# ZwwWayne/mmMOT

Hardware: AMD Instinct MI355X
Metric: frame-pairs/sec (fusion+affinity fwd) at N_det=64; affinity L∞ vs CPU ref (higher is better)
Workload: dtype f16x3

## Files before the change

include/mmmot_hip.h:

```cpp
#ifndef MMMOT_HIP_H
#define MMMOT_HIP_H

#include <stddef.h>
#include <stdint.h>

#ifdef __cplusplus
extern "C" {
#endif

#define MMMOT_OK 0
#define MMMOT_EINVAL (-1)

#define MMMOT_ACT_NONE 0
#define MMMOT_ACT_RELU 1
#define MMMOT_ACT_SIGMOID 2

#define MMMOT_A_PLAIN 0
#define MMMOT_A_NORM_RELU 1
#define MMMOT_A_PAIR 2

#define MMMOT_PAIR_MULTIPLY 0
#define MMMOT_PAIR_MINUS_ABS 1
#define MMMOT_PAIR_MINUS 2

// ... 101 lines not shown

int mmmot_gn_finalize(const float* part, const int* grp_tile0, const int* grp_ntiles,
                      const int* grp_count, const int* tile_nrows, int G, int ldp, int C, int NG,
                      const float* gamma, const float* beta, float eps,
                      float* sc, float* sh, void* stream);

int mmmot_segment_mean(const float* X, int ldx, int C,
                       const int* seg_start, const int* seg_count, const int* seg_stride,
                       const int* seg_group, const int* seg_div, int nseg,
                       const float* sc, const float* sh, int ldsc, int relu,
                       float* out, int ldo,
                       int hl16 ,
                       void* stream);

int mmmot_rowdot(const float* X, int ldx, int K, const float* w, float b,
                 const float* sc, const float* sh, int ldsc,
                 const int* tile_row0, const int* tile_nrows, const int* tile_group, int T,
                 int act, int use_thr, float thr,
                 float* out, const int* omap, void* stream);

int mmmot_row_layernorm(const float* X, int ldx, int C, const float* gamma, const float* beta,
                        float eps, int relu, float* Y, int ldy, int R, void* stream);

int mmmot_skippool_head(const float* P, int ldp, int C, int C4, const float* g0, const float* b0, const float* w1,
                        const float* c1, const float* g2, const float* b2, const float* w4, const float* c4,
                        const float* g5, const float* b5, float eps, float* out, int ldo, int R, void* stream);
int mmmot_pointnet_layer1(const float* X, int K, const float* W, const float* bias,
                          float* Y, float* part,
                          const int* tile_row0, const int* tile_nrows, int T, void* stream);

int mmmot_pn_mlp64(const float* X, int ldx, const float* sc, const float* sh, int ldsc, const void* W16,
                   float oscale, const float* bias, float* Y, int ldy, float* part, const int* tile_row0,
                   const int* tile_nrows, const int* tile_group, int T, int N, void* stream);

int mmmot_affine_act(const float* X, int ldx, int C, const float* sc, const float* sh, int ldsc,
                     const int* tile_row0, const int* tile_nrows, const int* tile_group, int T,
                     int act, float* Y, int ldy, void* stream);

int mmmot_fusion_combine(int mode, const float* cat, const float* Y0, int ld0,
                         const float* Y1, int ld1,
                         const float* sc0, const float* sh0, const float* sc1, const float* sh1, int ldsc,
                         const int* tile_row0, const int* tile_nrows, const int* tile_group, int T,
                         float* F, int Lt, int C, void* stream);

int mmmot_softmax_pairs(const float* logits, float* out,
                        const int* grp_row0, const int* grp_N, const int* grp_M, int G,
                        int max_nm ,
                        int mode, void* stream);

int mmmot_points_count(const float* pts, int P, int F, const double* planes, int NB, int pad_empty,
                       int* cnt, int* split, void* stream);
int mmmot_points_scatter(const float* pts, int P, int F, const double* planes, int NB, const int* cnt,
                         const int* split, float* out, int Fo, void* stream);
int mmmot_points_count_batched(const float* pts, int F, int NS, int NPOLY, int NBLK, int cnt_total,
                               const double* planes, const int* blk_sweep, const int* blk_first,
                               const int* sweep_row0, const int* poly0, const int* filt, const int* cnt_off,
                               int pad_empty, int* cnt, int* split, void* stream);
int mmmot_points_scatter_batched(const float* pts, int F, int NS, int NPOLY, int NBLK, int cnt_total,
                                 const double* planes, const int* blk_sweep, const int* blk_first,
                                 const int* sweep_row0, const int* poly0, const int* filt, const int* cnt_off,
                                 const int* cnt, const int* split, float* out, int Fo, void* stream);

int mmmot_u8_normalize(const unsigned char* u8, int N, int S, const float* mean_std, float* out, void* stream);
int mmmot_crop_resize_norm(const unsigned char* img, int H, int W, const int* boxes, int N, int S, int kmax,
                           const float* mean_std, int* work, float* out, unsigned char* out_u8, void* stream);

// ... 86 lines not shown
```

mmmot_amd/_lib.py:

```python
import ctypes
import os
import subprocess
import threading

_HERE = os.path.dirname(os.path.abspath(__file__))
CSRC = os.path.join(_HERE, 'csrc')
LIB_PATH = os.environ.get('MMMOT_LIB_PATH', os.path.join(_HERE, 'libmmmot_hip.so'))
SOURCES = ['conv3x3.hip', 'hl16_format.hip', 'conv3x3_hl16_patch.hip', 'gemm_rows.hip', 'gemm_wide.hip',
           'gemm_ares.hip', 'gemm_wres.hip', 'gemm_wreg.hip', 'pn_mlp64.hip', 'gram.hip', 'points_gather.hip', 'crop_resize.hip', 'small_kernels.hip', 'backward.hip', 'train.hip', 'train_vgg.hip', 'gemm_tn_f16.hip',
           'assign.hip', 'track_ids.hip']
HIPCC = os.environ.get('HIPCC', '/opt/rocm/bin/hipcc')
HIPFLAGS = ['--offload-arch=gfx950', '-O3', '-std=c++17', '-fPIC']

_lock = threading.Lock()
_lib = None

c_f = ctypes.c_void_p
c_i = ctypes.c_int


class GemmArgs(ctypes.Structure):
    _fields_ = [
        ('X', c_f), ('ldx', c_i),
        ('W', c_f),
        ('bias', c_f),
        ('dbias', c_f), ('rowidx', c_f), ('lddb', c_i),
        ('Y', c_f), ('ldy', c_i),
        ('part', c_f),
        ('sc', c_f), ('sh', c_f), ('ldsc', c_i),
        ('FA', c_f), ('FB', c_f), ('ldf', c_i),
        ('tile_row0', c_f), ('tile_nrows', c_f), ('tile_group', c_f),
        ('grp_row0', c_f), ('grp_M', c_f), ('grp_aoff', c_f), ('grp_boff', c_f),
        ('T', c_i), ('N', c_i), ('K', c_i),
        ('amode', c_i), ('pairop', c_i), ('act', c_i),
        ('w_hl16', c_i), ('oscale', ctypes.c_float),
        ('osc', c_f), ('osh', c_f), ('ldosc', c_i),
        ('colsum', c_f),
        ('pair_uniform32', c_i),
    ]


class GemmAresArgs(ctypes.Structure):
# ... 36 lines not shown
    'mmmot_gram_rows': [c_f, c_i, c_i, c_f, c_f, c_i, c_f, c_f, c_f, c_i, c_f, c_f, c_f],
    'mmmot_set_gram128_variant': [c_i],
    'mmmot_gn_finalize_gram': [c_f, c_f, c_f, c_f, c_f, c_i, c_i, c_f, c_f, c_i, c_f, c_f, ctypes.c_float, c_f, c_f, c_f, c_f],
    'mmmot_gn_finalize_gram_dbias': [c_f, c_f, c_f, c_f, c_f, c_i, c_f, c_f, c_i, c_f, c_f, c_i, c_i, c_f, c_f, ctypes.c_float,
                                     c_f, c_f, c_f, c_f],
    'mmmot_gn_finalize': [c_f, c_f, c_f, c_f, c_f, c_i, c_i, c_i, c_i, c_f, c_f, ctypes.c_float, c_f, c_f, c_f],
    'mmmot_segment_mean': [c_f, c_i, c_i, c_f, c_f, c_f, c_f, c_f, c_i, c_f, c_f, c_i, c_i, c_f, c_i, c_i, c_f],
    'mmmot_conv3x3_bn_relu_hl16_patch': [c_f, c_f, c_f, c_f, c_i, c_i, c_i, c_i, c_i, c_i, c_f, c_f],
    'mmmot_conv1_fused_hl16': [c_f, c_f, c_f, ctypes.c_float, c_f, c_f, c_f, c_f, c_i, c_i, c_i, c_f],
    'mmmot_conv3x3_bn_relu_hq8': [c_f, c_f, c_f, c_f, c_i, c_i, c_i, c_i, c_i, c_i, c_f, c_f],
    'mmmot_conv1_fused_u8': [c_f, ctypes.c_float, ctypes.c_float, ctypes.c_float, ctypes.c_float, ctypes.c_float,
                             ctypes.c_float, c_f, c_f, ctypes.c_float, c_f, c_f, c_f, c_f, c_i, c_i, c_i, c_i, c_f],
    'mmmot_u8_normalize': [c_f, c_i, c_i, c_f, c_f, c_f],
    'mmmot_conv1_fused_hq8': [c_f, c_f, c_f, ctypes.c_float, c_f, c_f, c_f, c_f, c_i, c_i, c_i, c_f],
    'mmmot_conv3x3_first_hl16': [c_f, c_f, c_f, c_f, c_i, c_i, c_i, c_i, c_f],
    'mmmot_set_patch_grid_limit': [c_i],
    'mmmot_set_patch_min_block': [c_i],
    'mmmot_trunk_range_read': [ctypes.POINTER(ctypes.c_uint), c_i],
    'mmmot_trunk_range_bind': [c_f],
    'mmmot_hl16_pack': [c_f, c_f, ctypes.c_long, c_f],
    'mmmot_hl16_unpack': [c_f, c_f, ctypes.c_long, c_f],
    'mmmot_hl16_pack_pow2': [c_f, c_f, ctypes.c_long, c_f, c_i, c_f],
    'mmmot_pow2_oscale': [c_f, c_i, c_f, c_i, c_f, c_i, c_f],
    'mmmot_conv3x3_raw_hl16': [c_f, c_f, c_f, c_f, c_i, c_i, c_i, c_i, c_i, c_f, c_f],
    'mmmot_hq8_pack': [c_f, c_f, ctypes.c_long, c_f],
    'mmmot_hq8_unpack': [c_f, c_f, ctypes.c_long, c_f],
    'mmmot_rowdot': [c_f, c_i, c_i, c_f, ctypes.c_float, c_f, c_f, c_i, c_f, c_f, c_f, c_i, c_i, c_i,
                     ctypes.c_float, c_f, c_f, c_f],
    'mmmot_row_layernorm': [c_f, c_i, c_i, c_f, c_f, ctypes.c_float, c_i, c_f, c_i, c_i, c_f],
    'mmmot_skippool_head': [c_f, c_i, c_i, c_i, c_f, c_f, c_f, c_f, c_f, c_f, c_f, c_f, c_f, c_f, ctypes.c_float, c_f, c_i, c_i,
                            c_f],
    'mmmot_pointnet_layer1': [c_f, c_i, c_f, c_f, c_f, c_f, c_f, c_f, c_i, c_f],
    'mmmot_pn_mlp64': [c_f, c_i, c_f, c_f, c_i, c_f, ctypes.c_float, c_f, c_f, c_i, c_f, c_f, c_f, c_f, c_i, c_i, c_f],
    'mmmot_affine_act': [c_f, c_i, c_i, c_f, c_f, c_i, c_f, c_f, c_f, c_i, c_i, c_f, c_i, c_f],
    'mmmot_fusion_combine': [c_i, c_f, c_f, c_i, c_f, c_i, c_f, c_f, c_f, c_f, c_i, c_f, c_f, c_f, c_i, c_f,
                             c_i, c_i, c_f],
    'mmmot_softmax_pairs': [c_f, c_f, c_f, c_f, c_f, c_i, c_i, c_i, c_f],
    'mmmot_points_count': [c_f, c_i, c_i, c_f, c_i, c_i, c_f, c_f, c_f],
    'mmmot_points_scatter': [c_f, c_i, c_i, c_f, c_i, c_f, c_f, c_f, c_i, c_f],
    'mmmot_crop_resize_norm': [c_f, c_i, c_i, c_f, c_i, c_i, c_i, c_f, c_f, c_f, c_f, c_f],
    'mmmot_points_count_batched': [c_f, c_i, c_i, c_i, c_i, c_i, c_f, c_f, c_f, c_f, c_f, c_f, c_f, c_i, c_f, c_f, c_f],
    'mmmot_points_scatter_batched': [c_f, c_i, c_i, c_i, c_i, c_i, c_f, c_f, c_f, c_f, c_f, c_f, c_f, c_f, c_f, c_f, c_i, c_f],
    'mmmot_selftest_mfma': [c_f, c_f, c_f, c_i, c_f],
    'mmmot_gn_bwd_partial': [c_f, c_i, c_f, c_i, c_i, c_f, c_f, c_i, c_f, c_f, c_i, c_f, c_f, c_f, c_i, c_f, c_f],
    'mmmot_gn_bwd_finalize': [c_f, c_f, c_i, c_i, c_i, c_f, c_f, c_f],
    'mmmot_gn_bwd_apply': [c_f, c_i, c_f, c_i, c_i, c_f, c_f, c_i, c_f, c_f, c_i, c_f, c_f, c_f, c_f, c_i, c_f, c_i, c_f],
    'mmmot_gemm_tn': [ctypes.POINTER(GemmTnArgs), c_f],
    'mmmot_gemm_tn_f16': [ctypes.POINTER(GemmTnArgs), c_f, c_f],
    'mmmot_absmax': [c_f, c_i, ctypes.c_long, c_i, c_f, c_f],
    'mmmot_pair_bwd': [c_f, c_i, c_f, c_i, c_f, c_i, c_i, c_f, c_f, c_f, c_f, c_f, c_f, c_f, c_i, c_i, c_i, c_f],
    'mmmot_pair_expand_bwd': [c_f, c_i, c_f, c_i, c_i, c_f, c_f, c_f, c_i, c_f, c_f, c_f, c_f, c_f],
    'mmmot_rowdot_bwd': [c_f, c_i, c_i, c_f, ctypes.c_float, c_f, c_f, c_i, c_f, c_f, c_f, c_i, c_i, c_f, c_f, c_f, c_i,
                         c_f, c_i, c_f],
    'mmmot_softmax_pairs_bwd': [c_f, c_f, c_f, c_f, c_f, c_f, c_i, c_i, c_i, c_f],
    'mmmot_fusion_c_bwd': [c_f, c_f, c_i, c_f, c_i, c_f, c_f, c_f, c_f, c_i, c_f, c_f, c_f, c_i, c_f, c_f, c_i, c_f, c_f, c_i, c_f],
    'mmmot_add_rows': [c_f, c_i, c_f, c_i, c_f, c_i, ctypes.c_long, c_i, c_f],
    'mmmot_conv3x3_raw': [c_f, c_f, c_f, c_f, c_i, c_i, c_i, c_i, c_i, c_i, c_f],
    'mmmot_rows_stats': [c_f, c_i, c_i, c_f, c_f, c_i, c_f, c_f],
    'mmmot_bn_relu_pool': [c_f, c_i, c_f, c_f, c_i, c_i, c_i, c_i, c_f, c_f],
    'mmmot_maxpool_bwd': [c_f, c_i, c_f, c_f, c_f, c_i, c_i, c_i, c_f, c_f],
    'mmmot_conv3x3_wgrad': [c_f, c_f, c_i, c_i, c_i, c_i, c_i, c_i, c_f, c_f],
    'mmmot_conv3x3_wgrad_f16': [c_f, c_f, c_i, c_i, c_i, c_i, c_i, c_i, c_f, c_f, c_f],
    'mmmot_conv3x3_first_wgrad': [c_f, c_f, c_i, c_i, c_i, c_f, c_i, c_f],
    'mmmot_rows_gather_scale': [c_f, c_i, c_f, c_f, c_f, c_i, ctypes.c_long, c_i, c_f],
    'mmmot_pointnet_layer1_bwd': [c_f, c_f, c_i, c_f, c_f, c_i, c_f, c_f],
    'mmmot_score_loss': [c_f, c_i, c_f, c_f, c_f, c_i, c_i, ctypes.c_float, c_i, ctypes.c_float, c_i, c_i, c_f, c_i, c_f,
# ... 74 lines not shown
```

mmmot_amd/engine.py:

```python
import contextlib
import itertools
import os
import threading

import numpy as np
import torch

from .ops import (ACT_NONE, ACT_RELU, ACT_SIGMOID, A_NORM_RELU, A_PAIR, A_PLAIN, FUSION_MODES, PAIR_OPS,
                  SOFTMAX_MODES)
from .range_guard import RangeGuard

POOL_INPUT = {'f32': 0, 'hl16': 1, 'hq8': 2}
EPS = 1e-5
_SERIALS = itertools.count(1)


def check_crop_side(S):
    if S < 32 or S % 2 != 0:
        raise ValueError('crop side %d is not supported: the HIP VGG trunk needs an even side >= 32; resize the crops '
                         '(mmmot_amd.crops.crop_resize_normalize)' % S)


def check_crop_layout(dets):
    if dets.dtype == torch.uint8:
        if dets.dim() != 4 or dets.shape[3] != 3 or dets.shape[1] != dets.shape[2]:
            raise ValueError('uint8 crops must be [L,S,S,3] (HWC, the output of mmmot_amd.crops.crop_resize_u8), got %s'
                             % (tuple(dets.shape),))
        S = int(dets.shape[1])
    else:
        S = int(dets.shape[-1])
    check_crop_side(S)
    return S


class Engine:
    def __init__(self, packed, ops, fusion='A', affinity_op='multiply', softmax_mode='none',
                 neg_threshold=0.0, score_arch='branch_cls', end_mode='avg', trunk=None):
        trunk = trunk or os.environ.get('MMMOT_TRUNK', 'f16x3')
        if trunk not in ('f16x3', 'f16q8', 'f32'):
            raise ValueError("trunk must be 'f16x3' (fp16 matrix cores, 3-term split), 'f16q8' (fp16 main term + "
                             "fp8 correction terms, include/mmmot_hip.h hq8) or 'f32' (exact fp32 MFMA)")
        self.trunk = trunk
        self.serial = next(_SERIALS)
        self.trunk_requested = trunk
        self.guard = RangeGuard(self)
        self.range_events = []
        self.last_out_of_range_forward = None
        self.out_of_range_window = None
        self._busy = threading.Lock()
        self._last_stream = None
        self._image_token = None
        self._pre_image = None
        ql = os.environ.get('MMMOT_Q8_LAYERS', '4,5,6,7,8,9,10,11,12')
        self.q8_layers = None if ql == 'all' else set(int(v) for v in ql.split(',') if v)
        self.pn_fused = os.environ.get('MMMOT_PN_FUSED', '1') != '0'
        self.pn_gram = os.environ.get('MMMOT_PN_GRAM', '1') != '0'
        self.pn_mlp64 = os.environ.get('MMMOT_PN_MLP64', '1') != '0'
        self.two_streams = os.environ.get('MMMOT_TWO_STREAMS', '0') == '1'
        self.pn_beside_trunk = os.environ.get('MMMOT_PN_BESIDE_TRUNK', '1') != '0'
        self._side = {}
        self.sp_fused = os.environ.get('MMMOT_SP_FUSED', '1') != '0'
        self.fuse_conv1 = os.environ.get('MMMOT_FUSE_CONV1', '1') != '0'
        self.q8_min_crop = int(os.environ.get('MMMOT_Q8_MIN_CROP', '64'))
        self.mlp = 'f32' if trunk == 'f32' else 'f16x3'
        if affinity_op not in PAIR_OPS:
            raise ValueError('unknown affinity_op %r' % (affinity_op,))
        if softmax_mode not in SOFTMAX_MODES and softmax_mode != 'none':
            softmax_mode = 'none'
        self.end_mode = end_mode
        self.P = packed
        self.ops = ops
        self.fusion = fusion
        self.affinity_op = affinity_op
        self.softmax_mode = softmax_mode
        self.neg_threshold = float(neg_threshold)
        self.score_arch = score_arch
        self.ws = {}
        self.dev = None
        self.keep = None
        self.conv_events = None

    def buf(self, name, *shape, device=None, dtype=torch.float32):
        n = 1
        for s in shape:
            n *= int(s)
        t = self.ws.get(name)
        if t is None or t.numel() < n or t.dtype != dtype or (device is not None and t.device != torch.device(device)):
            t = torch.empty(max(n, 4), dtype=dtype, device=device if device is not None else self.dev)
            self.ws[name] = t
        return t[:n].view(*shape)
# ... 137 lines not shown

    def _skippool(self, plan, s, x, hw, C, cat, fmt='f32'):
        hl16 = POOL_INPUT[fmt]
        ops, Lt, hd, T = self.ops, plan.Lt, self.P['skippool'][s], plan.det_tiles
        pooled = self.buf('sp_pool', Lt, C)
        first, second, npart = plan.crop_segments(hw)
        if second is None:
            ops.segment_mean(x, C, first, pooled, use_group=False, hl16=hl16)
        else:
            partial = self.buf('sp_partial', npart, C)
            ops.segment_mean(x, C, first, partial, use_group=False, hl16=hl16)
            ops.segment_mean(partial, C, second, pooled, use_group=False)
        if self.sp_fused and hasattr(ops, 'skippool_head'):
            ops.skippool_head(pooled, C, hd, EPS, cat[:, 128 * s:128 * (s + 1)], Lt)
            return
        ln0 = self.buf('sp_ln0', Lt, C)
        ops.row_layernorm(pooled, C, hd['g0'], hd['b0'], EPS, False, ln0, Lt)
        C4 = hd['w1'].shape[0]
        h1 = self.buf('sp_h1', Lt, C4)
        self._gemm(hd, 'w1', T, C4, C, X=ln0, bias=hd['c1'], Y=h1)
        ln1 = self.buf('sp_ln1', Lt, C4)
        ops.row_layernorm(h1, C4, hd['g2'], hd['b2'], EPS, True, ln1, Lt)
        h2 = self.buf('sp_h2', Lt, 128)
        self._gemm(hd, 'w4', T, 128, C4, X=ln1, bias=hd['c4'], Y=h2)
        ops.row_layernorm(h2, 128, hd['g5'], hd['b5'], EPS, True, cat[:, 128 * s:128 * (s + 1)], Lt)

    def pointnet(self, plan, points, cat):
        ops, pn, T, D, Pn, Lt = self.ops, self.P['pointnet'], plan.pt_tiles, plan.det_tiles, plan.P, plan.Lt
        y1 = self.buf('pn_y1', Pn, 64)
        part = self._part(T, 64)
        ops.pointnet_layer1(points, pn['w1'], pn['b1'], y1, part, T)
        sc1, sh1 = self._finalize('pn1', part, T, 64, 64, pn['g1'], pn['be1'])
        x, sc, sh = y1, sc1, sh1
        for i, (N, K) in zip((2, 3, 4), ((64, 64), (64, 64), (128, 64))):
            y = self.buf('pn_y%d' % i, Pn, N)
            part = self._part(T, N)
            if self.pn_mlp64 and self.mlp == 'f16x3' and ('w%d_h16' % i) in pn:
                ops.pn_mlp64(pn['w%d_h16' % i], pn['w%d_os' % i], T, N, x, sc, sh, pn['b%d' % i], y, part)
            else:
                self._gemm(pn, 'w%d' % i, T, N, K, X=x, bias=pn['b%d' % i], Y=y, part=part, sc=sc, sh=sh,
                           amode=A_NORM_RELU)
            sc, sh = self._finalize('pn%d' % i, part, T, N, N, pn['g%d' % i], pn['be%d' % i])
            x = y
        seg1024 = self._norm_relu_pool(plan, 'w5', '5', 128, 1024, x, sc, sh)
        self._stash('pn_seg1024', seg1024)
        dbias = self.buf('pn_dbias', Lt, 512)
        self._gemm(pn, 'wc1b', D, 512, 1024, X=seg1024, bias=pn['bc1'], Y=dbias)
        seg512 = self._norm_relu_pool(plan, 'wc1a', 'c1', 64, 512, y1, sc1, sh1, dbias=dbias)
        yc2, sc2, sh2 = self._gemm_gn(pn, 'wc2', D, 512, 512, 'pn_yc2', 'pnc2', 16, pn['gc2'], pn['bec2'], X=seg512,
                                      bias=pn['bc2'])
        ops.affine_act(yc2, 512, sc2, sh2, D, ACT_RELU, cat[:, 512:1024])

    def _norm_relu_pool(self, plan, w, s, K, N, x, sc, sh, dbias=None):
        ops, pn, T, Lt = self.ops, self.P['pointnet'], plan.pt_tiles, plan.Lt
        name, g, be = 'pn' + s, pn['g' + s], pn['be' + s]
        if dbias is None:
            ares_kw = row_kw = dict(bias=pn['b' + s])
        else:
            ares_kw, row_kw = dict(dbias=dbias, tile_dbrow=plan.tile_det), dict(dbias=dbias, rowidx=plan.row_det)
        seg = self.buf('pn_seg%d' % N, Lt, N)
        if self.pn_fused and self.mlp == 'f16x3' and (w + '_h16') in pn:
            TD, TH = plan.ptd_tiles, plan.ptd_half
            if self.pn_gram and (dbias is None or hasattr(ops, 'gn_finalize_gram_dbias')):
                GT, gram = (plan.gram_tiles, 'gram') if dbias is None else (plan.gram64_tiles, 'gram64')
                Gp, Sp = self.buf64(gram + '_G', GT.T, K * K), self.buf64(gram + '_S', GT.T, K)
                ops.gram_rows(x, K, sc, sh, GT, Gp, Sp)
                osc, osh = self.buf(name + '_sc', GT.G, N), self.buf(name + '_sh', GT.G, N)
                work = self.buf64(gram + '_work', GT.G, K * K + K)
                if dbias is None:
# ... 271 lines not shown
```

mmmot_amd/ops.py:

```python
import contextlib
import ctypes
import os
import threading

import torch

from . import _lib

ACT_NONE, ACT_RELU, ACT_SIGMOID = 0, 1, 2
A_PLAIN, A_NORM_RELU, A_PAIR = 0, 1, 2
PAIR_OPS = {'multiply': 0, 'minus_abs': 1, 'minus': 2}
SOFTMAX_MODES = {'single': 1, 'dual': 2, 'dual_add': 3, 'dual_max': 4}
FUSION_MODES = {'A': 0, 'B': 1, 'C': 2}
LOSS_KINDS = {'bce': 0, 'l2': 1, 'l1': 2}


def _ptr(t, dtype=torch.float32):
    if t is None:
        return None
    if not t.is_cuda:
        raise RuntimeError('mmmot_amd HIP ops need device tensors (got %s); there is no CPU fallback' % t.device)
    if t.dtype != dtype:
        raise TypeError('expected %s, got %s' % (dtype, t.dtype))
    return t.data_ptr()


def _iptr(t):
    return _ptr(t, torch.int32)


def _ld(t):
    if t is None:
        return 0
    if t.dim() == 1:
        return t.shape[0]
    if t.dim() != 2 or (t.shape[1] > 1 and t.stride(1) != 1):
        raise ValueError('expected a 2-D view with unit inner stride, got shape %s stride %s' % (
            tuple(t.shape), tuple(t.stride())))
    return t.stride(0)


class HipOps:
    name = 'hip'

    def __init__(self):
        self.lib = _lib.load()
        self._osvecs = {}
        self._scr = {}
        self.tn_f16 = os.environ.get('MMMOT_GEMM_TN', 'f16x3') != 'f32'
        self._tls = threading.local()

    @property
    def _pinned_stream(self):
        return getattr(self._tls, 'stream', None)

    @_pinned_stream.setter
    def _pinned_stream(self, v):
        self._tls.stream = v

    def _scratch(self, name, n, device):
        key = (name, n, str(device))
        t = self._scr.get(key)
        if t is None:
            t = self._scr[key] = torch.empty(n, dtype=torch.float32, device=device)
        return t

    def _osv(self, oscale, Cout, like):
        if torch.is_tensor(oscale):
            if oscale.numel() != Cout:
                raise ValueError('oscale must hold one scale per output channel')
            return oscale
        key = (float(oscale), Cout, like.device)
        v = self._osvecs.get(key)
        if v is None:
            v = self._osvecs[key] = torch.full((Cout,), float(oscale), dtype=torch.float32, device=like.device)
        return v

    def _stream(self):
        if self._pinned_stream is not None:
# ... 116 lines not shown
        a.FA, a.FB, a.ldf = _ptr(FA), _ptr(FB), _ld(FA)
        a.tile_row0, a.tile_nrows, a.tile_group = _iptr(tiles.row0), _iptr(tiles.nrows), _iptr(tiles.group)
        if pair is not None:
            a.grp_row0, a.grp_M = _iptr(pair['row0']), _iptr(pair['M'])
            a.grp_aoff, a.grp_boff = _iptr(pair['aoff']), _iptr(pair['boff'])
            a.pair_uniform32 = int(bool(pair.get('uniform32', False)))
        a.T, a.N, a.K = tiles.T, N, K
        a.amode, a.pairop, a.act = amode, pairop, act
        a.w_hl16, a.oscale = int(w_hl16), float(oscale)
        a.osc, a.osh, a.ldosc = _ptr(osc), _ptr(osh), _ld(osc)
        a.colsum = _ptr(colsum)
        _lib.check(self.lib.mmmot_gemm_rows(ctypes.byref(a), self._stream()), 'mmmot_gemm_rows')

    def gemm_ares(self, W16, oscale, tiles, N, K, X, sc, sh, bias=None, dbias=None, tile_dbrow=None, part=None,
                  osc=None, osh=None, colsum=None):
        a = _lib.GemmAresArgs()
        a.X, a.ldx = _ptr(X), _ld(X)
        a.sc, a.sh, a.ldsc = _ptr(sc), _ptr(sh), _ld(sc)
        a.W, a.bias = _ptr(W16), _ptr(bias)
        a.dbias, a.tile_dbrow, a.lddb = _ptr(dbias), _iptr(tile_dbrow), _ld(dbias)
        a.tile_row0, a.tile_nrows, a.tile_group = _iptr(tiles.row0), _iptr(tiles.nrows), _iptr(tiles.group)
        a.part = _ptr(part)
        a.osc, a.osh, a.ldosc = _ptr(osc), _ptr(osh), _ld(osc)
        a.colsum = _ptr(colsum)
        a.T, a.N, a.K, a.oscale = tiles.T, N, K, float(oscale)
        _lib.check(self.lib.mmmot_gemm_ares(ctypes.byref(a), self._stream()), 'mmmot_gemm_ares')

    def pn_mlp64(self, W16, oscale, tiles, N, X, sc, sh, bias, Y, part):
        st = self.lib.mmmot_pn_mlp64(_ptr(X), _ld(X), _ptr(sc), _ptr(sh), _ld(sc), _ptr(W16), float(oscale),
                                     _ptr(bias), _ptr(Y), _ld(Y), _ptr(part), _iptr(tiles.row0), _iptr(tiles.nrows),
                                     _iptr(tiles.group), tiles.T, N, self._stream())
        _lib.check(st, 'mmmot_pn_mlp64')

    def gram_rows(self, X, K, sc, sh, tiles, Gout, Sout):
        st = self.lib.mmmot_gram_rows(_ptr(X), _ld(X), K, _ptr(sc), _ptr(sh), _ld(sc), _iptr(tiles.row0),
                                      _iptr(tiles.nrows), _iptr(tiles.group), tiles.T,
                                      _ptr(Gout, torch.float64), _ptr(Sout, torch.float64), self._stream())
        _lib.check(st, 'mmmot_gram_rows')

    def gn_finalize_gram(self, Gp, Sp, tiles, K, W, bias, N, gamma, beta, eps, work, sc, sh):
        st = self.lib.mmmot_gn_finalize_gram(_ptr(Gp, torch.float64), _ptr(Sp, torch.float64), _iptr(tiles.g_tile0),
                                             _iptr(tiles.g_ntiles), _iptr(tiles.g_count), tiles.G, K, _ptr(W),
                                             _ptr(bias), N, _ptr(gamma), _ptr(beta), float(eps),
                                             _ptr(work, torch.float64), _ptr(sc), _ptr(sh), self._stream())
        _lib.check(st, 'mmmot_gn_finalize_gram')

    def gn_finalize_gram_dbias(self, Gp, Sp, tiles, tile_det, K, W, dbias, N, gamma, beta, eps, work, sc, sh):
        st = self.lib.mmmot_gn_finalize_gram_dbias(_ptr(Gp, torch.float64), _ptr(Sp, torch.float64), _iptr(tiles.g_tile0),
                                                   _iptr(tiles.g_ntiles), _iptr(tiles.g_count), tiles.G, _iptr(tiles.nrows),
                                                   _iptr(tile_det), K, _ptr(W), _ptr(dbias), _ld(dbias), N, _ptr(gamma),
                                                   _ptr(beta), float(eps), _ptr(work, torch.float64), _ptr(sc), _ptr(sh),
                                                   self._stream())
        _lib.check(st, 'mmmot_gn_finalize_gram_dbias')

    def gn_finalize(self, part, tiles, C, NG, gamma, beta, eps, sc, sh):
        if part.dim() != 3 or part.stride(2) != 1 or part.stride(0) != 2 * part.stride(1):
            raise ValueError('part must be a [T][2][C] view of a [T][2][ldp] buffer')
        st = self.lib.mmmot_gn_finalize(_ptr(part), _iptr(tiles.g_tile0), _iptr(tiles.g_ntiles),
                                        _iptr(tiles.g_count), _iptr(tiles.nrows) if tiles.ragged else None, tiles.G,
                                        part.stride(1), C, NG, _ptr(gamma), _ptr(beta),
                                        float(eps), _ptr(sc), _ptr(sh), self._stream())
        _lib.check(st, 'mmmot_gn_finalize')

    def segment_mean(self, X, C, segs, out, sc=None, sh=None, relu=False, use_group=True, hl16=False, take_max=False):
        st = self.lib.mmmot_segment_mean(_ptr(X), _ld(X), C, _iptr(segs.start), _iptr(segs.count),
                                         _iptr(segs.stride), _iptr(segs.group) if use_group else None,
# ... 191 lines not shown
```

mmmot_amd/profiler.py:

```python
import time

import torch

PEAK_F16X3_TFLOPS = 2500.0 / 3.0
PEAK_F32_TFLOPS = 157.3
PEAK_HBM_TBS = 8.0


def _rows(t):
    return int(getattr(t, 'R', 0))


def _seg_rows(segs):
    return int(segs.h_count.sum())


def _conv(name):
    def cost(a, k):
        inp, wp, bias, out, L, H, W, Cin, Cout = a[:9]
        pool = a[10] if name == 'conv3x3' else a[9]
        Ho, Wo = (H // 2, W // 2) if pool else (H, W)
        fl = 2.0 * L * H * W * 9 * Cin * Cout
        by = 4.0 * (L * H * W * Cin + L * Ho * Wo * Cout + 9 * Cin * Cout)
        return ('trunk conv %d->%d @%dx%d%s' % (Cin, Cout, H, W, ' +pool' if pool else ''), fl, by)
# ... 3 lines not shown
def _conv1_fused(a, k):
    i = max(j for j, v in enumerate(a) if torch.is_tensor(v))
    L, H, W = a[i + 1:i + 4]
    fl = 2.0 * L * H * W * 9 * (3 * 64 + 64 * 64)
    by = (1.0 if a[0].dtype == torch.uint8 else 4.0) * L * H * W * 3 + 4.0 * L * (H // 2) * (W // 2) * 64
    return ('trunk conv1_1+conv1_2 (fused) 3->64->64 @%dx%d +pool' % (H, W), fl, by)


def _gemm(a, k):
    W, tiles, N, K = a[:4]
    R = _rows(tiles)
    amode = k.get('amode', 0)
    kind = {0: 'plain', 1: 'norm+relu prologue', 2: 'pair prologue'}[amode]
    by = 4.0 * N * K + (4.0 * R * N if k.get('Y') is not None else 0.0)
    if amode != 2 and k.get('X') is not None:
        by += 4.0 * R * K
    if k.get('colsum') is not None or (k.get('Y') is None and k.get('part') is not None):
        kind += ', reduced'
    big = 'rows GEMM' if R >= 4096 else 'small GEMM'
    return ('%s %d->%d (%s)' % (big, K, N, kind), 2.0 * R * N * K, by)


def _gemm_ares(a, k):
    W16, oscale, tiles, N, K, X = a[:6]
    R = _rows(tiles)
    what = 'column sums' if k.get('colsum') is not None else 'statistics'
    return ('A-resident GEMM %d->%d (norm+relu prologue, %s only)' % (K, N, what), 2.0 * R * N * K, 4.0 * R * K + 4.0 * N * K)


def _pn_mlp64(a, k):
    W16, oscale, tiles, N = a[:4]
    R = _rows(tiles)
    return ('PointNet layer 64->%d (pn_mlp64)' % N, 2.0 * R * 64 * N, 4.0 * R * (64 + N))


def _gram(a, k):
    X, K, sc, sh, tiles = a[:5]
    R = _rows(tiles)
    return ('Gram matrix of the %d-channel rows (conv5 statistics)' % K, 2.0 * R * K * K, 4.0 * R * K)


def _segment_mean(a, k):
    X, C, segs, out = a[:4]
    R = _seg_rows(segs)
    kind = 'hl16 rows' if k.get('hl16') else ('norm+relu rows' if k.get('sc') is not None else 'rows')
    big = 'segment mean' if R >= 65536 else 'small segment mean'
    return ('%s, %d channels (%s)' % (big, C, kind), 1.0 * R * C, 4.0 * R * C)


def _rowdot(a, k):
    X, K, w, b, tiles, out = a[:6]
    R = _rows(tiles)
    return ('row dot %d->1' % K, 2.0 * R * K, 4.0 * R * K)


def _latency(label):
    return lambda a, k: (label, 0.0, 0.0)


def _layer1(a, k):
    X, W, bias, Y, part, tiles = a[:6]
    R = _rows(tiles)
    Kin = int(W.shape[1])
    return ('PointNet layer %d->64 (points in)' % Kin, 2.0 * R * Kin * 64, 4.0 * R * (Kin + 64))


COSTS = {
    'conv3x3': _conv('conv3x3'),
    'conv3x3_hl16_patch': _conv('hl16'),
    'conv3x3_hq8': _conv('hq8'),
    'conv1_fused_hl16': _conv1_fused,
    'conv1_fused_hq8': _conv1_fused,
    'conv1_fused_u8': _conv1_fused,
    'conv3x3_first_hl16': lambda a, k: ('trunk conv1_1 3->%d (fp32 MFMA)' % a[7], 2.0 * a[4] * a[5] * a[6] * 27 * a[7],
                                        4.0 * a[4] * a[5] * a[6] * (3 + a[7])),
    'gemm': _gemm,
    'gemm_ares': _gemm_ares,
    'pn_mlp64': _pn_mlp64,
    'gram_rows': _gram,
    'gn_finalize_gram': _latency('GroupNorm scale/shift from the Gram matrix'),
    'gn_finalize_gram_dbias': _latency('GroupNorm scale/shift from the Gram matrix'),
    'gn_finalize': _latency('GroupNorm scale/shift from tile partials'),
    'segment_mean': _segment_mean,
    'rowdot': _rowdot,
    'row_layernorm': _latency('row LayerNorm'),
    'skippool_head': _latency('SkipPool head (LN, 1x1, LN, 1x1, LN)'),
    'pointnet_layer1': _layer1,
    'affine_act': _latency('affine + activation rows'),
    'fusion_combine': _latency('fusion combine'),
    'softmax_pairs': _latency('pair softmax'),
    'u8_normalize': _latency('8-bit crops -> fp32'),
    'hq8_pack': _latency('hq8 / hl16 re-encode'), 'hq8_unpack': _latency('hq8 / hl16 re-encode'),
    'hl16_pack': _latency('hq8 / hl16 re-encode'), 'hl16_unpack': _latency('hq8 / hl16 re-encode'),
}


class LaunchProfiler:

    def __init__(self, ops, f32=False):
        self.ops = ops
        self.cuda = torch.cuda.is_available()
        self.peak_tf = PEAK_F32_TFLOPS if f32 else PEAK_F16X3_TFLOPS
        self.records = []
        self._saved = {}

    def _wrap(self, name, fn, cost):
        def wrapped(*a, **k):
            try:
                label, fl, by = cost(a, k)
            except Exception:
                label, fl, by = name, 0.0, 0.0
# ... 74 lines not shown
```

Measured before the change: 312.4.

## Fuse PointNet MLP chain into one recompute-from-points kernel per layer

Adds a pn_chain kernel that recomputes PointNet layers from the raw points inside one kernel, keeping activations in LDS as split f16 hi/lo pairs and running f16x3 MFMA, so intermediate activations are not written to or read back from global memory. Because GroupNorm statistics must be finalized between layers, it is launched three times with depth 1, 2 and 3, recomputing the earlier layers each time. Only the last depth stores its output, and the layer-1 launch is kept. This trades redundant MFMA compute for less HBM traffic on intermediate activations.

```diff
diff --git a/include/mmmot_hip.h b/include/mmmot_hip.h
--- a/include/mmmot_hip.h
+++ b/include/mmmot_hip.h
@@ -157,6 +157,11 @@
 int mmmot_pn_mlp64(const float* X, int ldx, const float* sc, const float* sh, int ldsc, const void* W16,
                    float oscale, const float* bias, float* Y, int ldy, float* part, const int* tile_row0,
                    const int* tile_nrows, const int* tile_group, int T, int N, void* stream);
+
+int mmmot_pn_chain(const float* P, int K, const float* W1, const float* b1, int depth, const float* const* sc,
+                   const float* const* sh, int ldsc, const void* const* W16, const float* oscale,
+                   const float* const* bias, float* Y, int ldy, float* part, const int* tile_row0,
+                   const int* tile_nrows, const int* tile_group, int T, void* stream);
 
 int mmmot_affine_act(const float* X, int ldx, int C, const float* sc, const float* sh, int ldsc,
                      const int* tile_row0, const int* tile_nrows, const int* tile_group, int T,
diff --git a/mmmot_amd/_lib.py b/mmmot_amd/_lib.py
--- a/mmmot_amd/_lib.py
+++ b/mmmot_amd/_lib.py
@@ -7,7 +7,7 @@
 CSRC = os.path.join(_HERE, 'csrc')
 LIB_PATH = os.environ.get('MMMOT_LIB_PATH', os.path.join(_HERE, 'libmmmot_hip.so'))
 SOURCES = ['conv3x3.hip', 'hl16_format.hip', 'conv3x3_hl16_patch.hip', 'gemm_rows.hip', 'gemm_wide.hip',
-           'gemm_ares.hip', 'gemm_wres.hip', 'gemm_wreg.hip', 'pn_mlp64.hip', 'gram.hip', 'points_gather.hip', 'crop_resize.hip', 'small_kernels.hip', 'backward.hip', 'train.hip', 'train_vgg.hip', 'gemm_tn_f16.hip',
+           'gemm_ares.hip', 'gemm_wres.hip', 'gemm_wreg.hip', 'pn_mlp64.hip', 'pn_chain.hip', 'gram.hip', 'points_gather.hip', 'crop_resize.hip', 'small_kernels.hip', 'backward.hip', 'train.hip', 'train_vgg.hip', 'gemm_tn_f16.hip',
            'assign.hip', 'track_ids.hip']
 HIPCC = os.environ.get('HIPCC', '/opt/rocm/bin/hipcc')
 HIPFLAGS = ['--offload-arch=gfx950', '-O3', '-std=c++17', '-fPIC']
@@ -110,6 +110,7 @@
                             c_f],
     'mmmot_pointnet_layer1': [c_f, c_i, c_f, c_f, c_f, c_f, c_f, c_f, c_i, c_f],
     'mmmot_pn_mlp64': [c_f, c_i, c_f, c_f, c_i, c_f, ctypes.c_float, c_f, c_f, c_i, c_f, c_f, c_f, c_f, c_i, c_i, c_f],
+    'mmmot_pn_chain': [c_f, c_i, c_f, c_f, c_i, c_f, c_f, c_i, c_f, c_f, c_f, c_f, c_i, c_f, c_f, c_f, c_f, c_i, c_f],
     'mmmot_affine_act': [c_f, c_i, c_i, c_f, c_f, c_i, c_f, c_f, c_f, c_i, c_i, c_f, c_i, c_f],
     'mmmot_fusion_combine': [c_i, c_f, c_f, c_i, c_f, c_i, c_f, c_f, c_f, c_f, c_i, c_f, c_f, c_f, c_i, c_f,
                              c_i, c_i, c_f],
diff --git a/mmmot_amd/csrc/pn_chain.hip b/mmmot_amd/csrc/pn_chain.hip
--- /dev/null
+++ b/mmmot_amd/csrc/pn_chain.hip
@@ -0,0 +1,286 @@
+#include "common.h"
+
+#define PC_K 64
+#define PC_LDT 72
+
+struct pc_layer {
+  const float* sc;
+  const float* sh;
+  const u32x4* W16;
+  const float* bias;
+  float oscale;
+};
+struct pc_args {
+  pc_layer L[3];
+};
+
+template <int KIN, int DEPTH, bool STORE>
+__global__ __launch_bounds__(256, DEPTH == 3 ? 1 : 2) void pn_chain_kernel(const float* __restrict__ P, const float* __restrict__ W1,
+                                                       const float* __restrict__ b1, const pc_args a, int ldsc,
+                                                       float* __restrict__ Y, int ldy, float* __restrict__ part,
+                                                       const int* __restrict__ tile_row0,
+                                                       const int* __restrict__ tile_nrows,
+                                                       const int* __restrict__ tile_group, int T) {
+  constexpr int NLAST = DEPTH == 3 ? 128 : 64;
+  constexpr int WROWS = DEPTH == 3 ? 256 : 64 * DEPTH;
+  constexpr int NI = DEPTH > 1 ? DEPTH - 1 : 1;
+  __shared__ __attribute__((aligned(16))) _Float16 Wh[WROWS * PC_LDT];
+  __shared__ __attribute__((aligned(16))) _Float16 Wl[WROWS * PC_LDT];
+  __shared__ __attribute__((aligned(16))) _Float16 Ah[MM_BM * PC_LDT];
+  __shared__ __attribute__((aligned(16))) _Float16 Al[MM_BM * PC_LDT];
+  __shared__ float red[2][4][NLAST];
+  __shared__ float xs[MM_BM * KIN];
+  const int tid = threadIdx.x, lane = tid & 63, wave = tid >> 6;
+  const int lr = lane & 31, kh = (lane >> 5) * 8;
+
+#pragma unroll
+  for (int j = 0; j < DEPTH; ++j) {
+    const int nj = j == 2 ? 128 : 64;
+    for (int idx = tid; idx < nj * 8; idx += 256) {
+      const int n = idx >> 3, u = idx & 7;
+      const u32x4 hi = a.L[j].W16[(long)idx * 2], lo = a.L[j].W16[(long)idx * 2 + 1];
+      *reinterpret_cast<u32x4*>(&Wh[(j * 64 + n) * PC_LDT + u * 8]) = hi;
+      *reinterpret_cast<u32x4*>(&Wl[(j * 64 + n) * PC_LDT + u * 8]) = lo;
+    }
+  }
+  const int srow = tid >> 4, sc0 = (tid & 15) * 4;
+  float w1[4][KIN], bv1[4];
+#pragma unroll
+  for (int e = 0; e < 4; ++e) {
+#pragma unroll
+    for (int k = 0; k < KIN; ++k) w1[e][k] = W1[(sc0 + e) * KIN + k];
+    bv1[e] = b1[sc0 + e];
+  }
+  float px[2];
+  f32x4 s0, h0;
+  float sjn[NI][2], hjn[NI][2], bj[NI][2];
+#pragma unroll
+  for (int j = 0; j < DEPTH - 1; ++j)
+#pragma unroll
+    for (int nt = 0; nt < 2; ++nt) bj[j][nt] = a.L[j].bias ? a.L[j].bias[nt * 32 + lr] : 0.f;
+  auto load_tile = [&](int tt) {
+    const int row0 = tile_row0[tt], nw = tile_nrows[tt] * KIN;
+    const long go = (long)(tile_group ? tile_group[tt] : 0) * ldsc;
+#pragma unroll
+    for (int q = 0; q < 2; ++q) {
+      const int idx = tid + 256 * q;
+      px[q] = idx < nw ? P[(long)row0 * KIN + idx] : 0.f;
+    }
+    s0 = *reinterpret_cast<const f32x4*>(a.L[0].sc + go + sc0);
+    h0 = *reinterpret_cast<const f32x4*>(a.L[0].sh + go + sc0);
+#pragma unroll
+    for (int j = 0; j < DEPTH - 1; ++j)
+#pragma unroll
+      for (int nt = 0; nt < 2; ++nt) {
+        sjn[j][nt] = a.L[j + 1].sc[go + nt * 32 + lr];
+        hjn[j][nt] = a.L[j + 1].sh[go + nt * 32 + lr];
+      }
+  };
+  auto put_points = [&]() {
+#pragma unroll
+    for (int q = 0; q < 2; ++q) {
+      const int idx = tid + 256 * q;
+      if (idx < MM_BM * KIN) xs[idx] = px[q];
+    }
+  };
+  int t = blockIdx.x;
+  if (t < T) {
+    load_tile(t);
+    put_points();
+  }
+  float bv[NLAST / 32];
+#pragma unroll
+  for (int nt = 0; nt < NLAST / 32; ++nt) bv[nt] = a.L[DEPTH - 1].bias ? a.L[DEPTH - 1].bias[nt * 32 + lr] : 0.f;
+  __syncthreads();
+
+  for (; t < T; t += gridDim.x) {
+    const int row0 = tile_row0[t], nrows = tile_nrows[t];
+    float sj[NI][2], hj[NI][2];
+#pragma unroll
+    for (int j = 0; j < DEPTH - 1; ++j)
+#pragma unroll
+      for (int nt = 0; nt < 2; ++nt) sj[j][nt] = sjn[j][nt], hj[j][nt] = hjn[j][nt];
+    {
+#pragma unroll
+      for (int i = 0; i < 8; ++i) {
+        const int r = srow + 16 * i;
+        float p[KIN];
+#pragma unroll
+        for (int k = 0; k < KIN; ++k) p[k] = xs[r * KIN + k];
+        float y[4];
+#pragma unroll
+        for (int e = 0; e < 4; ++e) {
+          float v = bv1[e];
+#pragma unroll
+          for (int k = 0; k < KIN; ++k) v = fmaf(w1[e][k], p[k], v);
+          y[e] = fminf(fmaxf(fmaf(v, s0[e], h0[e]), 0.f), 65000.f);
+          if (r >= nrows) y[e] = 0.f;
+        }
+        unsigned h0_, l0_, h1_, l1_;
+        mm_split2(y[0], y[1], h0_, l0_);
+        mm_split2(y[2], y[3], h1_, l1_);
+        *reinterpret_cast<u32x2*>(&Ah[r * PC_LDT + sc0]) = u32x2{h0_, h1_};
+        *reinterpret_cast<u32x2*>(&Al[r * PC_LDT + sc0]) = u32x2{l0_, l1_};
+      }
+    }
+    const int tn = t + gridDim.x;
+    if (tn < T) load_tile(tn);
+    __syncthreads();
+    bool valid[16];
+#pragma unroll
+    for (int e = 0; e < 16; ++e) valid[e] = wave * 32 + mm_acc_row(e, lane) < nrows;
+    const int offa = (wave * 32 + lr) * PC_LDT + kh;
+
+#pragma unroll
+    for (int j = 0; j < DEPTH - 1; ++j) {
+      f32x16 acc[2];
+#pragma unroll
+      for (int nt = 0; nt < 2; ++nt)
+#pragma unroll
+        for (int e = 0; e < 16; ++e) acc[nt][e] = 0.f;
+#pragma unroll
+      for (int ks = 0; ks < PC_K / 16; ++ks) {
+        const f16x8 ah = *reinterpret_cast<const f16x8*>(&Ah[offa + ks * 16]);
+        const f16x8 al = *reinterpret_cast<const f16x8*>(&Al[offa + ks * 16]);
+#pragma unroll
+        for (int nt = 0; nt < 2; ++nt) {
+          const int offb = (j * 64 + nt * 32 + lr) * PC_LDT + kh + ks * 16;
+          const f16x8 bh = *reinterpret_cast<const f16x8*>(&Wh[offb]);
+          const f16x8 bl = *reinterpret_cast<const f16x8*>(&Wl[offb]);
+          acc[nt] = __builtin_amdgcn_mfma_f32_32x32x16_f16(al, bh, acc[nt], 0, 0, 0);
+          acc[nt] = __builtin_amdgcn_mfma_f32_32x32x16_f16(ah, bl, acc[nt], 0, 0, 0);
+          acc[nt] = __builtin_amdgcn_mfma_f32_32x32x16_f16(ah, bh, acc[nt], 0, 0, 0);
+        }
+      }
+      const float osc = a.L[j].oscale;
+#pragma unroll
+      for (int nt = 0; nt < 2; ++nt) {
+        const int n = nt * 32 + lr;
+#pragma unroll
+        for (int e = 0; e < 16; e += 2) {
+          float y[2];
+#pragma unroll
+          for (int q = 0; q < 2; ++q) {
+            const float v = fmaf(acc[nt][e + q], osc, bj[j][nt]);
+            y[q] = fminf(fmaxf(fmaf(v, sj[j][nt], hj[j][nt]), 0.f), 65000.f);
+            if (!valid[e + q]) y[q] = 0.f;
+          }
+          unsigned h2, l2;
+          mm_split2(y[0], y[1], h2, l2);
+          const f16x2 hh = __builtin_bit_cast(f16x2, h2), ll = __builtin_bit_cast(f16x2, l2);
+#pragma unroll
+          for (int q = 0; q < 2; ++q) {
+            const int o = (wave * 32 + mm_acc_row(e + q, lane)) * PC_LDT + n;
+            Ah[o] = hh[q];
+            Al[o] = ll[q];
+          }
+        }
+      }
+      __syncthreads();
+    }
+
+    constexpr int NT = NLAST / 32;
+    constexpr int JL = DEPTH - 1;
+    f32x16 acc[NT];
+#pragma unroll
+    for (int nt = 0; nt < NT; ++nt)
+#pragma unroll
+      for (int e = 0; e < 16; ++e) acc[nt][e] = 0.f;
+#pragma unroll
+    for (int ks = 0; ks < PC_K / 16; ++ks) {
+      const f16x8 ah = *reinterpret_cast<const f16x8*>(&Ah[offa + ks * 16]);
+      const f16x8 al = *reinterpret_cast<const f16x8*>(&Al[offa + ks * 16]);
+#pragma unroll
+      for (int nt = 0; nt < NT; ++nt) {
+        const int offb = (JL * 64 + nt * 32 + lr) * PC_LDT + kh + ks * 16;
+        const f16x8 bh = *reinterpret_cast<const f16x8*>(&Wh[offb]);
+        const f16x8 bl = *reinterpret_cast<const f16x8*>(&Wl[offb]);
+        acc[nt] = __builtin_amdgcn_mfma_f32_32x32x16_f16(al, bh, acc[nt], 0, 0, 0);
+        acc[nt] = __builtin_amdgcn_mfma_f32_32x32x16_f16(ah, bl, acc[nt], 0, 0, 0);
+        acc[nt] = __builtin_amdgcn_mfma_f32_32x32x16_f16(ah, bh, acc[nt], 0, 0, 0);
+      }
+    }
+    const float oscale = a.L[JL].oscale;
+#pragma unroll
+    for (int nt = 0; nt < NT; ++nt) {
+      float s1 = 0.f;
+#pragma unroll
+      for (int e = 0; e < 16; ++e) {
+        acc[nt][e] = fmaf(acc[nt][e], oscale, bv[nt]);
+        if (valid[e]) {
+          s1 += acc[nt][e];
+          if (STORE) Y[(long)(row0 + wave * 32 + mm_acc_row(e, lane)) * ldy + nt * 32 + lr] = acc[nt][e];
+        }
+      }
+      s1 = mm_xor32_sum(s1);
+      if (lane < 32) red[0][wave][nt * 32 + lr] = s1;
+    }
+    __syncthreads();
+    const float inv = 1.f / (float)nrows;
+#pragma unroll
+    for (int nt = 0; nt < NT; ++nt) {
+      const int n = nt * 32 + lr;
+      const float tot = red[0][0][n] + red[0][1][n] + red[0][2][n] + red[0][3][n];
+      const float mu = tot * inv;
+      float s2 = 0.f;
+#pragma unroll
+      for (int e = 0; e < 16; ++e) {
+        const float d = acc[nt][e] - mu;
+        if (valid[e]) s2 = fmaf(d, d, s2);
+      }
+      s2 = mm_xor32_sum(s2);
+      if (lane < 32) red[1][wave][n] = s2;
+      if (wave == 0 && lane < 32) part[((long)t * 2 + 0) * NLAST + n] = tot;
+    }
+    if (tn < T) put_points();
+    __syncthreads();
+    if (wave == 0 && lane < 32) {
+#pragma unroll
+      for (int nt = 0; nt < NT; ++nt) {
+        const int n = nt * 32 + lr;
+        part[((long)t * 2 + 1) * NLAST + n] = red[1][0][n] + red[1][1][n] + red[1][2][n] + red[1][3][n];
+      }
+    }
+  }
+}
+
+template <int KIN>
+static void pc_launch(int depth, int grid, hipStream_t s, const float* P, const float* W1, const float* b1,
+                      const pc_args& a, int ldsc, float* Y, int ldy, float* part, const int* tile_row0,
+                      const int* tile_nrows, const int* tile_group, int T) {
+  if (depth == 1)
+    hipLaunchKernelGGL((pn_chain_kernel<KIN, 1, false>), dim3(grid), dim3(256), 0, s, P, W1, b1, a, ldsc, Y, ldy, part,
+                       tile_row0, tile_nrows, tile_group, T);
+  else if (depth == 2)
+    hipLaunchKernelGGL((pn_chain_kernel<KIN, 2, false>), dim3(grid), dim3(256), 0, s, P, W1, b1, a, ldsc, Y, ldy, part,
+                       tile_row0, tile_nrows, tile_group, T);
+  else
+    hipLaunchKernelGGL((pn_chain_kernel<KIN, 3, true>), dim3(grid), dim3(256), 0, s, P, W1, b1, a, ldsc, Y, ldy, part,
+                       tile_row0, tile_nrows, tile_group, T);
+}
+
+extern "C" int mmmot_pn_chain(const float* P, int K, const float* W1, const float* b1, int depth, const float* const* sc,
+                              const float* const* sh, int ldsc, const void* const* W16, const float* oscale,
+                              const float* const* bias, float* Y, int ldy, float* part, const int* tile_row0,
+                              const int* tile_nrows, const int* tile_group, int T, void* stream) {
+  if (!P || !W1 || !b1 || !sc || !sh || !W16 || !oscale || !bias || !part || !tile_row0 || !tile_nrows || T <= 0)
+    return MMMOT_EINVAL;
+  if ((K != 3 && K != 4) || depth < 1 || depth > 3 || ldsc % 4 != 0 || ldsc < 64) return MMMOT_EINVAL;
+  if (depth == 3 && (!Y || ldy < 128)) return MMMOT_EINVAL;
+  pc_args a;
+  for (int j = 0; j < 3; ++j) {
+    const int i = j < depth ? j : 0;
+    if (!sc[i] || !sh[i] || !W16[i] || !mm_al16(sc[i]) || !mm_al16(sh[i]) || !mm_al16(W16[i])) return MMMOT_EINVAL;
+    a.L[j] = pc_layer{sc[i], sh[i], (const u32x4*)W16[i], bias[i], oscale[i]};
+  }
+  const int n_cu = mm_num_cu();
+  if (n_cu <= 0) return MMMOT_EINVAL;
+  const int per_cu = depth == 3 ? 1 : 2;
+  const int grid = T < per_cu * n_cu ? T : per_cu * n_cu;
+  hipStream_t s = (hipStream_t)stream;
+  if (K == 3)
+    pc_launch<3>(depth, grid, s, P, W1, b1, a, ldsc, Y, ldy, part, tile_row0, tile_nrows, tile_group, T);
+  else
+    pc_launch<4>(depth, grid, s, P, W1, b1, a, ldsc, Y, ldy, part, tile_row0, tile_nrows, tile_group, T);
+  return mm_check(hipGetLastError());
+}
diff --git a/mmmot_amd/engine.py b/mmmot_amd/engine.py
--- a/mmmot_amd/engine.py
+++ b/mmmot_amd/engine.py
@@ -56,6 +56,7 @@
         self.pn_fused = os.environ.get('MMMOT_PN_FUSED', '1') != '0'
         self.pn_gram = os.environ.get('MMMOT_PN_GRAM', '1') != '0'
         self.pn_mlp64 = os.environ.get('MMMOT_PN_MLP64', '1') != '0'
+        self.pn_chain = os.environ.get('MMMOT_PN_CHAIN', '1') != '0'
         self.two_streams = os.environ.get('MMMOT_TWO_STREAMS', '0') == '1'
         self.pn_beside_trunk = os.environ.get('MMMOT_PN_BESIDE_TRUNK', '1') != '0'
         self._side = {}
@@ -259,9 +260,19 @@
         ops.pointnet_layer1(points, pn['w1'], pn['b1'], y1, part, T)
         sc1, sh1 = self._finalize('pn1', part, T, 64, 64, pn['g1'], pn['be1'])
         x, sc, sh = y1, sc1, sh1
+        chain = hasattr(ops, 'pn_chain') and self.pn_chain and self.pn_mlp64 and self.mlp == 'f16x3' and \
+            all(('w%d_h16' % i) in pn for i in (2, 3, 4))
+        layers = []
         for i, (N, K) in zip((2, 3, 4), ((64, 64), (64, 64), (128, 64))):
+            part = self._part(T, N)
+            if chain:
+                layers.append((pn['w%d_h16' % i], pn['w%d_os' % i], sc, sh, pn['b%d' % i]))
+                y = self.buf('pn_y4', Pn, N) if i == 4 else None
+                ops.pn_chain(points, pn['w1'], pn['b1'], layers, T, y, part)
+                sc, sh = self._finalize('pn%d' % i, part, T, N, N, pn['g%d' % i], pn['be%d' % i])
+                x = y
+                continue
             y = self.buf('pn_y%d' % i, Pn, N)
-            part = self._part(T, N)
             if self.pn_mlp64 and self.mlp == 'f16x3' and ('w%d_h16' % i) in pn:
                 ops.pn_mlp64(pn['w%d_h16' % i], pn['w%d_os' % i], T, N, x, sc, sh, pn['b%d' % i], y, part)
             else:
diff --git a/mmmot_amd/ops.py b/mmmot_amd/ops.py
--- a/mmmot_amd/ops.py
+++ b/mmmot_amd/ops.py
@@ -45,6 +45,8 @@
 
     def __init__(self):
         self.lib = _lib.load()
+        if hasattr(self.lib, 'mmmot_pn_chain'):
+            self.pn_chain = self._pn_chain
         self._osvecs = {}
         self._scr = {}
         self.tn_f16 = os.environ.get('MMMOT_GEMM_TN', 'f16x3') != 'f32'
@@ -227,6 +229,16 @@
                                      _iptr(tiles.group), tiles.T, N, self._stream())
         _lib.check(st, 'mmmot_pn_mlp64')
 
+    def _pn_chain(self, points, W1, b1, layers, tiles, Y, part):
+        depth = len(layers)
+        arr = ctypes.c_void_p * depth
+        W16s, scs, shs, bs = (arr(*[_ptr(l[i]) for l in layers]) for i in (0, 2, 3, 4))
+        oscs = (ctypes.c_float * depth)(*[float(l[1]) for l in layers])
+        st = self.lib.mmmot_pn_chain(_ptr(points), int(W1.shape[1]), _ptr(W1), _ptr(b1), depth, scs, shs, _ld(layers[0][2]),
+                                     W16s, oscs, bs, _ptr(Y), _ld(Y), _ptr(part), _iptr(tiles.row0), _iptr(tiles.nrows),
+                                     _iptr(tiles.group), tiles.T, self._stream())
+        _lib.check(st, 'mmmot_pn_chain')
+
     def gram_rows(self, X, K, sc, sh, tiles, Gout, Sout):
         st = self.lib.mmmot_gram_rows(_ptr(X), _ld(X), K, _ptr(sc), _ptr(sh), _ld(sc), _iptr(tiles.row0),
                                       _iptr(tiles.nrows), _iptr(tiles.group), tiles.T,
diff --git a/mmmot_amd/profiler.py b/mmmot_amd/profiler.py
--- a/mmmot_amd/profiler.py
+++ b/mmmot_amd/profiler.py
@@ -59,6 +59,16 @@
     W16, oscale, tiles, N = a[:4]
     R = _rows(tiles)
     return ('PointNet layer 64->%d (pn_mlp64)' % N, 2.0 * R * 64 * N, 4.0 * R * (64 + N))
+
+
+def _pn_chain(a, k):
+    points, W1, b1, layers, tiles, Y = a[:6]
+    R, depth, Kin = _rows(tiles), len(layers), int(W1.shape[1])
+    N = 128 if depth == 3 else 64
+    fl = 2.0 * R * (Kin * 64 + 64 * 64 * min(depth, 2) + (64 * 128 if depth == 3 else 0))
+    by = 4.0 * R * (Kin + (N if Y is not None else 0))
+    return ('PointNet layers %d->64%s->%d from the points (pn_chain, depth %d)' % (Kin, '->64' * (min(depth, 2) - (depth < 3)),
+                                                                                 N, depth), fl, by)
 
 
 def _gram(a, k):
@@ -104,6 +114,7 @@
     'gemm': _gemm,
     'gemm_ares': _gemm_ares,
     'pn_mlp64': _pn_mlp64,
+    'pn_chain': _pn_chain,
     'gram_rows': _gram,
     'gn_finalize_gram': _latency('GroupNorm scale/shift from the Gram matrix'),
     'gn_finalize_gram_dbias': _latency('GroupNorm scale/shift from the Gram matrix'),
```

New measurement: 309.6. Within noise of the previous version (-0.9%).
